# worm-privacy/proof-of-burn

Measured on NVIDIA H100. Metric: main_proof_of_burn witnesses/sec, higher is better.
Workload: dtype u256 (BN254-Fr integer)

## Files before the change

proof-of-burn_b200/csrc/compiler.cpp:

```cpp
#include "compiler.h"
#include <sys/mman.h>
#include <algorithm>
#include <array>
#include <cstdlib>
#include <cstring>
#include <stdexcept>
#include <unordered_map>
#include "poseidon_constants_data.h"
#include "r1cs.h"
#include "vm_exec.h"

namespace pob {
namespace {

struct Blk { uint64_t sig; size_t pos; };
struct Lane { uint32_t w; };

static const Code ZERO = 0, ONE = 1;

struct KeyHash {
    size_t operator()(const std::array<uint32_t, 4> &k) const {
        uint64_t h = 0x9E3779B97F4A7C15ULL;
        for (uint32_t v : k) { h ^= v; h *= 0xBF58476D1CE4E5B9ULL; h ^= h >> 29; }
        return (size_t)h;
// ... 2003 lines not shown
        for (size_t i = 0; i < B.flat_n; i++) B.flat[i] = rc(B.flat[i]);
    }
    std::vector<uint32_t> round_keep;
    if (opt_level) {
        const uint64_t N = B.nsig;
        EqClasses E = eq_classes(P, N);
        const uint64_t n_io = 1ull + n_out + n_in;
        auto kept = [&](uint64_t s) { if (s < n_io) return true; const uint32_t r = E.root((uint32_t)s); return r == s && !E.is_const_root[r]; };
        if (!B.round_sigs.empty()) { const uint64_t b0 = B.round_sigs[0]; for (uint32_t i = 0; i < ROUND_SIGNALS; i++) if (kept(b0 + i)) round_keep.push_back(i); }
        P.witness_map.reserve(N / 8);
        for (auto &sg : B.segs) {
            if (sg.round) {
                size_t k = 0;
                for (uint32_t i = 0; i < ROUND_SIGNALS; i++) {
                    const bool kp = kept(sg.dst + i);
                    const bool want = k < round_keep.size() && round_keep[k] == i;
                    if (kp != want) throw std::runtime_error("pob: internal: KeccakfRound blocks do not reduce uniformly");
                    if (kp) { P.witness_map.push_back((uint32_t)(sg.dst + i)); k++; }
                }
            } else for (uint64_t i = 0; i < sg.n; i++) if (kept(sg.dst + i)) P.witness_map.push_back((uint32_t)(sg.dst + i));
        }
    }
    P.codes.resize(ROUND_SIGNALS);
    { LaneSink S{P.codes.data(), 0}; emit_round(S);
      if ((size_t)(S.p - P.codes.data()) != ROUND_SIGNALS) throw std::runtime_error("pob: internal: round table size mismatch"); }
    P.round_desc = derive_round_desc(P.codes.data(), ROUND_SIGNALS);
    P.n_round_blocks = B.n_round_blocks; P.n_flat_signals = B.flat_n; P.n_signals_o0 = B.nsig; P.opt_level = opt_level;
    if (opt_level) {
        std::vector<Code> rt(round_keep.size()); for (size_t k = 0; k < round_keep.size(); k++) rt[k] = P.codes[round_keep[k]];
        P.codes = rt;
        const uint32_t RT = (uint32_t)round_keep.size();
        bool fast_round = true;
        try { P.round_desc = derive_round_desc(rt.data(), RT); } catch (const std::exception &) { fast_round = false; P.round_desc.assign(1, 0); }
        if (P.round_desc.empty()) P.round_desc.assign(1, 0);
        P.out_code_off = RT + 1;
        uint64_t dst = 0; size_t mp = 0;
        const uint32_t ts = TILE_SIGNALS;
        for (auto &sg : B.segs) {
            if (sg.round) {
                const uint32_t rts = (fast_round && RT <= MAX_TILE_SIGNALS) ? RT : ts;
                for (uint32_t done = 0; done < RT; done += rts) { Tile t; t.dst = dst + done; t.n = std::min(rts, RT - done); t.code_off = done; t.ubase = sg.ubase; t.pad = fast_round ? 1 : 0; P.tiles.push_back(t); }
                dst += RT; mp += RT;
            } else {
                const size_t first = P.codes.size();
                while (mp < P.witness_map.size() && P.witness_map[mp] < sg.dst + sg.n) { P.codes.push_back(B.flat[sg.pos + (P.witness_map[mp] - sg.dst)]); mp++; }
                const uint64_t n = P.codes.size() - first;
                for (uint64_t done = 0; done < n; done += ts) { Tile t; t.dst = dst + done; t.n = (uint32_t)std::min<uint64_t>(ts, n - done); t.code_off = (uint32_t)(first + done); t.ubase = 0; t.pad = 0; P.tiles.push_back(t); }
                dst += n;
            }
        }
        if (dst != P.witness_map.size() || mp != P.witness_map.size()) throw std::runtime_error("pob: internal: reduced layout does not add up");
        P.n_signals = dst;
        if (!user_wants_constraints) { P.cons_flat = ConsSet(); P.cons_round = ConsSet(); P.has_constraints = false; }
        std::stable_sort(P.tiles.begin(), P.tiles.end(), [](const Tile &a, const Tile &b) { return a.pad > b.pad; });
        return P;
    }
    P.codes.insert(P.codes.end(), B.flat, B.flat + B.flat_n);
    uint32_t tile_signals = LAYOUT_TILE_SIGNALS;
#ifdef POB_TUNING
    if (const char *v = getenv("POB_TILE_SIGNALS")) { uint32_t t = (uint32_t)atoi(v); if (t >= 128 && t <= TILE_SIGNALS && t % 128 == 0) tile_signals = t; }
#endif
    for (auto &s : B.segs) {
        uint64_t done = 0;
        while (done < s.n) {
            uint32_t n = (uint32_t)std::min<uint64_t>(tile_signals, s.n - done);
            Tile t; t.dst = s.dst + done; t.n = n; t.pad = 0;
            if (s.round) { t.code_off = (uint32_t)done; t.ubase = s.ubase; t.pad = 1; }
            else { t.code_off = (uint32_t)(ROUND_SIGNALS + s.pos + done); t.ubase = 0; }
            P.tiles.push_back(t); done += n;
        }
    }
    std::stable_sort(P.tiles.begin(), P.tiles.end(), [](const Tile &a, const Tile &b) { return a.pad > b.pad; });
    return P;
}

static uint64_t lc_key(uint32_t idx, bool rel) { return idx == CONS_ONE ? 0 : rel ? (uint64_t)idx + 1 : idx; }
static uint64_t lc_idx(uint64_t key, bool rel) { return !rel ? key : key == 0 ? CONS_ONE : key - 1; }
static LC lc_of(const ConsTerm *t, uint32_t n, const std::vector<Fr> &konst, bool rel) {
    LC L; for (uint32_t i = 0; i < n; i++) L.sf(lc_key(t[i].idx, rel), cons_coef_value(t[i].coef, konst.data(), 0)); return L;
}
static void lc_normalize(LC &L) {
    std::sort(L.t.begin(), L.t.end(), [](const std::pair<uint64_t, Fr> &x, const std::pair<uint64_t, Fr> &y) { return x.first < y.first; });
    size_t o = 0;
    for (size_t i = 0; i < L.t.size();) {
        std::pair<uint64_t, Fr> m = L.t[i++];
        while (i < L.t.size() && L.t[i].first == m.first) m.second = fr_add(m.second, L.t[i++].second);
        if (!fr_is_zero(m.second)) L.t[o++] = m;
    }
    L.t.resize(o);
}
static void lc_unkey(LC &L, bool rel) { for (auto &q : L.t) q.first = lc_idx(q.first, rel); }
static bool plan_r1(ConsSink &S, LC &A, LC &Bq, LC &C, bool rel) {
    lc_normalize(A); lc_normalize(Bq); lc_normalize(C);
    if (A.t.empty()) Bq.t.clear();
    if (A.t.empty() && C.t.empty()) return false;
    lc_unkey(A, rel); lc_unkey(Bq, rel); lc_unkey(C, rel);
    S.r1(A, Bq, C);
    return true;
}

static void plan_o0_set(const ConsSet &in, ConsSink &S, bool rel) {
    const std::vector<Fr> &konst = *S.konst;
    for (size_t i = 0; i + 1 < in.eq.size(); i += 2) if (in.eq[i] != in.eq[i + 1]) S.eq(in.eq[i], in.eq[i + 1]);
    for (const ConsTerm &t : in.kc) {
        const bool on_one = t.idx == CONS_ONE || (!rel && t.idx == 0);
        if (on_one && cc_kind(t.coef) != CC_RCBIT && fr_eq(cons_coef_value(t.coef, konst.data(), 0), fr_from_u64(1))) continue;
        S.kc_raw(t.idx, t.coef);
    }
    for (const ConsR1 &r : in.r1) {
        if (r1_hint(r)) continue;
        const ConsTerm *t = in.terms.data() + r.off;
        LC A = lc_of(t, r.na, konst, rel), Bq = lc_of(t + r.na, r.nb, konst, rel), C = lc_of(t + r.na + r.nb, r1_nc(r), konst, rel);
        plan_r1(S, A, Bq, C, rel);
    }
}

static uint64_t plan_set_terms(const ConsSet &S, const std::vector<Fr> &konst, bool rel, uint64_t rc) {
    uint64_t n = S.eq.size();
    for (const ConsTerm &t : S.kc) {
        const bool on_one = t.idx == CONS_ONE || (!rel && t.idx == 0);
        n += (on_one || fr_is_zero(cons_coef_value(t.coef, konst.data(), rc))) ? 1 : 2;
    }
    for (const ConsR1 &r : S.r1) n += r.na + r.nb + r1_nc(r);
    return n;
}
// ... 127 lines not shown
```

proof-of-burn_b200/csrc/kernels.cuh:

```cuda
#pragma once
#include <cuda_runtime.h>
#include "vm_exec.h"
#include "cons_check.h"

using namespace pob;

namespace {

__constant__ uint64_t c_keccak_rc[24] = {
    0x0000000000000001ULL, 0x0000000000008082ULL, 0x800000000000808AULL, 0x8000000080008000ULL, 0x000000000000808BULL,
    0x0000000080000001ULL, 0x8000000080008081ULL, 0x8000000000008009ULL, 0x000000000000008AULL, 0x0000000000000088ULL,
    0x0000000080008009ULL, 0x000000008000000AULL, 0x000000008000808BULL, 0x800000000000008BULL, 0x8000000000008089ULL,
    0x8000000000008003ULL, 0x8000000000008002ULL, 0x8000000000000080ULL, 0x000000000000800AULL, 0x800000008000000AULL,
    0x8000000080008081ULL, 0x8000000000008080ULL, 0x0000000080000001ULL, 0x8000000080008008ULL};
__constant__ int c_keccak_rot[25] = {1, 10, 7, 11, 17, 18, 3, 5, 16, 8, 21, 24, 4, 15, 23, 19, 13, 12, 2, 20, 14, 22, 9, 6, 1};
__constant__ int c_keccak_inv_rot[25] = {0, 23, 17, 5, 11, 6, 22, 1, 8, 21, 0, 2, 16, 15, 19, 12, 7, 3, 4, 14, 18, 9, 20, 13, 10};

__device__ void absorb_warp(uint64_t *W, const AbsorbOp op) {
    const unsigned FULL = 0xffffffffu;
    const int lane = threadIdx.x & 31;
    const bool act = lane < 25;
    const int l = act ? lane : 0;
    uint64_t st = (act && op.s_idx != NONE_IDX) ? W[op.s_idx + l] : 0ull;
    if (lane < 17) st ^= W[op.blk_idx + lane];
// ... 216 lines not shown
            for (; i < L.t_end; i += GT) {
                const Op cur = nxt;
                if (i + GT < L.t_end) { nxt = ldg_op(a.ops + i + GT); if (a.prefetch) prefetch_operands(x, nxt); }
                vm_exec_op(x, cur);
            }
        }
        for (uint32_t q = L.p_begin + gwarp; q < L.p_end; q += nwarp) poseidon_warp(x, a.poseidons[q], s_pk);
        { const uint32_t np = (L.p_end - L.p_begin) % nwarp, wv = (gwarp + nwarp - np) % nwarp;
          for (uint32_t w = L.w_begin + wv; w < L.w_end; w += nwarp) absorb_warp(U, a.absorbs[w]);
          const uint32_t nw2 = (np + (L.w_end - L.w_begin)) % nwarp, sv = (gwarp + nwarp - nw2) % nwarp;
          for (uint32_t q = L.s_begin + sv; q < L.s_end; q += nwarp) psum_warp(x, a.psums[q]); }
        if (inv_worker) {
            if (lv == a.ginv_level) {
                InvChain c;
                if (vm_ginv_start(x, a.ops, a.ginv_begin, a.inv_end, wid, NWK, c)) { inv_park(s_inv, INV_WORKERS, wt, c); inv_running = true; }
            } else if (inv_running) {
                InvChain c = inv_unpark(s_inv, INV_WORKERS, wt);
                if (inv_chain_steps(c, INV_STEPS)) { vm_ginv_finish(x, a.ops, a.ginv_begin, a.inv_end, wid, NWK, inv_chain_result(c)); inv_running = false; }
                else inv_park(s_inv, INV_WORKERS, wt, c);
            }
        }
        cluster_sync_all();
    }
    if (a.prof && inst == 0 && gt == 0) a.prof[a.n_levels] = clock64();
    if (inv_worker) {
        if (a.ginv_level >= a.n_levels) vm_inv_batch(x, a.ops, a.ginv_begin, a.inv_end, wid, NWK);
        else if (inv_running) {
            InvChain c = inv_unpark(s_inv, INV_WORKERS, wt);
            while (!inv_chain_steps(c, 64)) { }
            vm_ginv_finish(x, a.ops, a.ginv_begin, a.inv_end, wid, NWK, inv_chain_result(c));
        }
    }
    if (a.prof && inst == 0) { cluster_sync_all(); if (gt == 0) { a.prof[a.n_levels + 1] = clock64(); a.prof[a.n_levels + 2] = clock64(); } }
    __syncthreads();
    if (tid == 0 && s_status != STATUS_OK) atomicMin(a.status + inst, s_status);
    cluster_sync_all();
    if (gt == 0 && atomicAdd(a.status + inst, 0u) == STATUS_OK) a.status[inst] = 0u;
    for (uint32_t i = gt; i < a.n_outputs; i += GT) {
        uint64_t v[4]; vm_expand(a.out_codes[i], U, 0, a.val_base, a.konst, v);
        uint64_t *o = a.outputs + ((uint64_t)inst * a.n_outputs + i) * 4;
        o[0] = v[0]; o[1] = v[1]; o[2] = v[2]; o[3] = v[3];
    }
}

__device__ __forceinline__ void st128(uint64_t *p, uint64_t a, uint64_t b) { asm volatile("st.global.v2.b64 [%0], {%1, %2};" ::"l"(p), "l"(a), "l"(b)); }

struct ExpandArgs {
    const Tile *tiles; const Code *codes; const Fr *konst; const uint2 *round_desc;
    const uint64_t *stores; uint64_t store_stride; uint32_t val_base;
    uint64_t *const *wit;
    const uint32_t *inst;
    const uint32_t *status;
    uint32_t chunk_first;
    uint32_t tile0;
};

constexpr int ROUND_THREADS = 256;
__global__ void __launch_bounds__(ROUND_THREADS) k_expand_round(const ExpandArgs a) {
    const uint32_t gi = a.inst[blockIdx.y];
    if (a.status[gi] != 0) return;
    const Tile t = a.tiles[blockIdx.x];
    const uint64_t *Ub = a.stores + (uint64_t)(gi - a.chunk_first) * a.store_stride + t.ubase;
    uint64_t *W = a.wit[blockIdx.y] + t.dst * 4;
    __shared__ __align__(16) uint2 sD[MAX_TILE_SIGNALS / 64];
    __shared__ __align__(16) uint64_t sWraw[ROUND_WORDS_SPAN + 3];
    __shared__ __align__(8) uint64_t s_bar;
    const uint32_t odd = (uint32_t)((reinterpret_cast<uintptr_t>(Ub) >> 3) & 1u);
    const uint32_t nd = (t.n + 63) >> 6, d_bytes = ((nd + 1) & ~1u) * 8u, w_bytes = (ROUND_WORDS_SPAN + 3) / 2 * 16u;
    if (threadIdx.x == 0) mbar_init(&s_bar, 1);
    __syncthreads();
    if (threadIdx.x == 0) {
        mbar_expect_tx(&s_bar, d_bytes + w_bytes);
        tma_load_1d(sD, a.round_desc + (t.code_off >> 6), d_bytes, &s_bar);
        tma_load_1d(sWraw, Ub - odd, w_bytes, &s_bar);
    }
    mbar_wait(&s_bar, 0);
    const uint64_t *sW = sWraw + odd;
#pragma unroll 8
    for (uint32_t u = threadIdx.x; u < 2 * t.n; u += ROUND_THREADS) {
        const uint32_t k = u >> 1;
        const uint2 d = sD[k >> 6];
        const uint32_t tt = k & 63, mode = d.y >> 16;
        uint32_t w = d.x & 0xffffu, b = tt;
        if (mode) {
            const uint32_t sidx = (mode - 1) * 64 + tt, g = sidx / 3, m = sidx - 3 * g;
            b = g; w = (m == 0) ? (d.x & 0xffffu) : (m == 1) ? (d.x >> 16) : (d.y & 0xffffu);
        }
        const uint64_t v = (u & 1u) ? 0ull : (sW[w] >> b) & 1ull;
        st128(W + 2ull * u, v, 0);
    }
}

__global__ void __launch_bounds__(256, 3) k_expand_codes(const ExpandArgs a) {
    constexpr int UG = 4;
    const uint32_t gi = a.inst[blockIdx.x];
    if (a.status[gi] != 0) return;
    const Tile t = a.tiles[a.tile0 + blockIdx.y];
    const uint64_t *U = a.stores + (uint64_t)(gi - a.chunk_first) * a.store_stride;
    uint64_t *W = a.wit[blockIdx.x] + t.dst * 4;
    const uint64_t *Ub = U + t.ubase;
    __shared__ __align__(16) Code sC[TILE_SIGNALS + 4];
    __shared__ __align__(8) uint64_t s_bar;
    const uint32_t off4 = t.code_off & 3u, bytes = (((t.n + off4) * 4u) + 15u) & ~15u;
    if (threadIdx.x == 0) mbar_init(&s_bar, 1);
    __syncthreads();
    if (threadIdx.x == 0) { mbar_expect_tx(&s_bar, bytes); tma_load_1d(sC, a.codes + (t.code_off - off4), bytes, &s_bar); }
    mbar_wait(&s_bar, 0);
    const Code *c = sC + off4;
    const uint32_t n2 = 2 * t.n, h = threadIdx.x & 1u;
    for (uint32_t base = threadIdx.x; base < n2; base += 256 * UG) {
        uint64_t v[UG][2];
#pragma unroll
        for (int j = 0; j < UG; j++) {
            const uint32_t u = base + 256 * j;
            const Code cd = u < n2 ? c[u >> 1] : 0u;
            const uint32_t kind = code_kind(cd), p = code_payload(cd);
            v[j][0] = v[j][1] = 0;
            if (kind == K_VAL || kind == K_KONST) {
                const uint64_t *s = (kind == K_VAL) ? U + a.val_base + 4ull * p : reinterpret_cast<const uint64_t *>(a.konst + p);
                const ulonglong2 q = reinterpret_cast<const ulonglong2 *>(s)[h];
                v[j][0] = q.x; v[j][1] = q.y;
            } else if (!h) v[j][0] = (kind == K_BIT) ? (Ub[p >> 6] >> (p & 63)) & 1ull : p;
        }
#pragma unroll
        for (int j = 0; j < UG; j++) { const uint32_t u = base + 256 * j; if (u < n2) st128(W + 2ull * u, v[j][0], v[j][1]); }
    }
}

__global__ void __launch_bounds__(256) k_digest(const uint64_t *wit, uint64_t n_signals, unsigned long long *out, const uint32_t *status) {
    if (status && *status != 0) return;
    uint64_t acc = 0;
    for (uint64_t i = (uint64_t)blockIdx.x * blockDim.x + threadIdx.x; i < n_signals; i += (uint64_t)gridDim.x * blockDim.x) {
        const ulonglong4 v = *reinterpret_cast<const ulonglong4 *>(wit + 4 * i);
        uint64_t h = (i + 1) * 0x9E3779B97F4A7C15ULL;
        h ^= v.x * 0xBF58476D1CE4E5B9ULL + v.y * 0x94D049BB133111EBULL + v.z * 0xD6E8FEB86659FD93ULL + v.w * 0xA0761D6478BD642FULL;
        h ^= h >> 29; h *= 0xBF58476D1CE4E5B9ULL; h ^= h >> 32;
        acc += h;
    }
    for (int o = 16; o > 0; o >>= 1) acc += __shfl_down_sync(0xffffffffu, acc, o);
    __shared__ uint64_t part[8];
    if ((threadIdx.x & 31) == 0) part[threadIdx.x >> 5] = acc;
    __syncthreads();
    if (threadIdx.x == 0) { uint64_t s = 0; for (int w = 0; w < 8; w++) s += part[w]; atomicAdd(out, (unsigned long long)s); }
}

struct GrindArgs { uint64_t start[4], lanes_tail[9]; uint64_t first, count; uint32_t zero_bytes; unsigned long long *hit; };
__device__ __forceinline__ uint64_t bswap64(uint64_t x) { return __byte_perm((uint32_t)(x >> 32), 0, 0x0123) | ((uint64_t)__byte_perm((uint32_t)x, 0, 0x0123) << 32); }
__device__ __forceinline__ uint64_t rotl64(uint64_t x, int n) { return (x << n) | (x >> (64 - n)); }
__global__ void __launch_bounds__(256) k_pow_grind(const GrindArgs a) {
    const uint64_t idx = (uint64_t)blockIdx.x * blockDim.x + threadIdx.x;
    if (idx >= a.count) return;
    uint64_t k0 = a.start[0], k1 = a.start[1], k2 = a.start[2], k3 = a.start[3];
    const uint64_t add = a.first + idx;
    k0 += add; if (k0 < add) { if (++k1 == 0) { if (++k2 == 0) ++k3; } }
    uint64_t s[25];
    s[0] = bswap64(k3); s[1] = bswap64(k2); s[2] = bswap64(k1); s[3] = bswap64(k0);
#pragma unroll
    for (int i = 0; i < 9; i++) s[4 + i] = a.lanes_tail[i];
    s[13] = 0x01; s[14] = 0; s[15] = 0; s[16] = 0x8000000000000000ull;
#pragma unroll
    for (int i = 17; i < 25; i++) s[i] = 0;
#pragma unroll 1
    for (int r = 0; r < 24; r++) {
        uint64_t c[5], d[5], b[25];
#pragma unroll
        for (int x = 0; x < 5; x++) c[x] = s[x] ^ s[x + 5] ^ s[x + 10] ^ s[x + 15] ^ s[x + 20];
#pragma unroll
        for (int x = 0; x < 5; x++) d[x] = c[(x + 4) % 5] ^ rotl64(c[(x + 1) % 5], 1);
#pragma unroll
        for (int i = 0; i < 25; i++) s[i] ^= d[i % 5];
        b[0] = s[0];
#pragma unroll
        for (int i = 0; i < 24; i++) b[keccak_rot(i + 1)] = rotl64(s[keccak_rot(i)], keccak_shl(i));
#pragma unroll
        for (int i = 0; i < 25; i++) s[i] = b[i] ^ (~b[chi_b(i)] & b[chi_c(i)]);
        s[0] ^= c_keccak_rc[r];
    }
    const uint64_t mask = a.zero_bytes >= 8 ? ~0ull : ((1ull << (8 * a.zero_bytes)) - 1);
    if ((s[0] & mask) == 0) atomicMin(a.hit, (unsigned long long)idx);
// ... 112 lines not shown
```

proof-of-burn_b200/csrc/pob_b200.cu:

```cuda
#include <cuda.h>
#include <cuda_runtime.h>
#include <fcntl.h>
#include <unistd.h>
#include <algorithm>
#include <chrono>
#include <condition_variable>
#include <cstdio>
#include <cstdlib>
#include <cstring>
#include <deque>
#include <mutex>
#include <stdexcept>
#include <string>
#include <thread>
#include <vector>
#include "../../include/pob_b200.h"
#include "compiler.h"
#include "kernels.cuh"
#include "ntt.cuh"
#include "r1cs.h"

using namespace pob;

static thread_local std::string g_err;
// ... 87 lines not shown
        }
    }
    int grab() {
        std::unique_lock<std::mutex> l(m);
        const int b = next_b; cv.wait(l, [&] { return !busy[b]; });
        busy[b] = true; next_b = (b + 1) % NB; return b;
    }
    void drain() { std::unique_lock<std::mutex> l(m); cv.wait(l, [this] { if (!q.empty()) return false; for (int i = 0; i < NB; i++) if (busy[i]) return false; return true; }); }
    static size_t header(uint8_t *o, uint64_t n) {
        uint32_t u32; uint64_t u64; Fr p = fr_p(); size_t k = 0;
        auto put = [&](const void *s, size_t b) { memcpy(o + k, s, b); k += b; };
        put("wtns", 4); u32 = 2; put(&u32, 4); u32 = 2; put(&u32, 4);
        u32 = 1; put(&u32, 4); u64 = 40; put(&u64, 8); u32 = 32; put(&u32, 4); put(p.l, 32); u32 = (uint32_t)n; put(&u32, 4);
        u32 = 2; put(&u32, 4); u64 = 32ull * n; put(&u64, 8);
        return k;
    }
    void send(const uint64_t *dwit, uint64_t n_signals, int fd) {
        CU(cudaSetDevice(device));
        if (fd >= 0) { uint8_t hd[80]; size_t hb = header(hd, n_signals); if (pwrite(fd, hd, hb, 0) != (ssize_t)hb) { std::lock_guard<std::mutex> l(m); io_err = true; } }
        const uint64_t total = 32ull * n_signals; const uint64_t nch = (total + bb - 1) / bb;
        for (uint64_t c = 0; c < nch; c++) {
            const uint64_t off = c * bb; const size_t bytes = (size_t)std::min<uint64_t>(bb, total - off);
            const int b = grab(); cudaStream_t s = cs[rr++ % NS];
            CU(cudaMemcpyAsync(buf[b], (const char *)dwit + off, bytes, cudaMemcpyDeviceToHost, s));
            CU(cudaEventRecord(ev[b], s));
            { std::lock_guard<std::mutex> l(m); q.push_back(Job{b, fd, 76 + off, bytes, c + 1 == nch}); }
            cv.notify_all();
            bytes_moved += bytes;
        }
        if (nch == 0 && fd >= 0) close(fd);
        for (int i = 1; i < NS; i++) { CU(cudaEventRecord(ev_join, cs[i])); CU(cudaStreamWaitEvent(cs[0], ev_join, 0)); }
    }
};

}

struct pob_handle {
    Program P; int device = 0; uint32_t n_sms = 0;
    Op *d_ops = nullptr; PsumOp *d_psums = nullptr; PoseidonOp *d_pos = nullptr; Fr *d_pos_konst = nullptr; AbsorbOp *d_abs = nullptr; Level *d_levels = nullptr; Code *d_aux = nullptr; Fr *d_konst = nullptr;
    Code *d_codes = nullptr; Tile *d_tiles = nullptr; Fr *d_invtab = nullptr; uint64_t *d_round_desc = nullptr;
    static const uint32_t RING = 2;
    uint32_t chunk = 0; uint64_t store_stride = 0; uint64_t *d_stores = nullptr; uint64_t *d_inputs = nullptr;
    std::vector<uint64_t *> slots;
    std::vector<VmSlot> slot_vm; size_t slot_bytes = 0; uint32_t n_compressed_slots = 0;
    std::vector<int64_t> slot_owner;
    std::vector<cudaEvent_t> slot_rel_ev; std::vector<uint8_t> slot_rel_pending;
    std::vector<uint32_t> last_status; uint32_t last_n = 0;
    uint32_t cap_n = 0; uint32_t *d_status = nullptr; uint64_t *d_outputs = nullptr; unsigned long long *d_digests = nullptr;
    uint64_t **d_witptr = nullptr; uint32_t *d_planinst = nullptr;
    uint32_t *h_status = nullptr; uint64_t *h_outputs = nullptr; uint64_t *h_digests = nullptr; uint64_t **h_witptr = nullptr; uint32_t *h_planinst = nullptr;
    uint64_t *d_staged = nullptr; uint32_t n_staged = 0;
    long long *d_prof = nullptr; std::string prof_path;
    uint32_t xgroup = 0;
    uint32_t n_round_tiles = 0;
    uint64_t *d_block_base = nullptr; uint32_t n_blocks = 0;
    uint32_t round_dyn_smem = 85 * 1024;
    uint32_t codes_dyn_smem = 24 * 1024;
    int eval_threads = 512; uint32_t eval_cluster = 0, eval_prefetch = 0;
    uint32_t pos_konst_bytes = 0, levels_bytes = 0, eval_smem = 0;
    bool skip_eval = false;
    cudaStream_t s_eval = nullptr, s_exp = nullptr, s_h2d = nullptr;
    cudaEvent_t ev_eval_done[RING] = {nullptr, nullptr}, ev_exp_done[RING] = {nullptr, nullptr}, ev_h2d[RING] = {nullptr, nullptr},
                ev_start = nullptr, ev_end = nullptr, ev_tmp = nullptr;
    std::vector<cudaEvent_t> ev_pool; size_t ev_used = 0;
    struct Group { uint32_t begin, end, chunk; cudaEvent_t t0, t1; };
    struct Batch {
        bool active = false, async = false, staged = false, digest = false;
        const uint64_t *inputs = nullptr; uint32_t n = 0, nchunks = 0, next_eval = 0, next_group = 0, acq_pos = 0;
        std::vector<uint32_t> plan, slot;
        std::vector<uint8_t> st;
        std::vector<cudaStream_t> acq_stream;
        std::vector<uint32_t> group_of;
        std::vector<Group> groups; std::vector<uint32_t> chunk_gend;
        std::vector<cudaEvent_t> e0, e1, est;
        pob_timing T{};
    } B;
    Exporter *exporter = nullptr;
    pob_timing timing{};
    struct DevCons {
        bool ready = false; ConsView flat{}, round{}; Fr *konst = nullptr; uint64_t *bases = nullptr; uint32_t n_blocks = 0;
        unsigned long long *rep = nullptr; std::vector<void *> allocs; pob_check_report info{};
    } cons, r1cs;
    struct DevNtt { bool ready = false; uint32_t log_n = 0; NttTables t{}; std::vector<void *> allocs; } ntt;
};

static void cons_info(const Program &P, pob_check_report *r) {
    memset(r, 0, sizeof *r);
    const uint64_t nb = P.round_block_sig.size();
    auto count = [&](const ConsSet &S, uint64_t mult) {
        r->n_constraints += mult * (S.eq.size() / 2 + S.kc.size());
        for (const ConsR1 &q : S.r1) { if (r1_hint(q)) r->n_hints += mult; else { r->n_constraints += mult; if (q.na) r->n_nonlinear += mult; } }
    };
    count(P.cons_flat, 1); count(P.cons_round, nb);
    std::vector<uint8_t> seen(P.n_signals, 0);
    auto mark = [&](const ConsSet &S, uint64_t base) {
        for (uint32_t i : S.eq) seen[base + i] = 1;
        for (const ConsTerm &t : S.kc) seen[base + t.idx] = 1;
        for (const ConsTerm &t : S.terms) if (t.idx != CONS_ONE) seen[base + t.idx] = 1;
    };
    mark(P.cons_flat, 0);
    for (uint64_t b : P.round_block_sig) mark(P.cons_round, b);
    for (uint8_t v : seen) r->signals_read += v;
    r->first_failed = ~0ull;
}
static ConsView upload_cons(pob_handle::DevCons &C, const ConsSet &S) {
    ConsView v{};
    auto up = [&](const void *src, size_t bytes) { void *d = nullptr; CU(cudaMalloc(&d, std::max<size_t>(16, bytes))); if (bytes) CU(cudaMemcpy(d, src, bytes, cudaMemcpyHostToDevice)); C.allocs.push_back(d); return d; };
    v.eq = (const uint32_t *)up(S.eq.data(), S.eq.size() * 4); v.n_eq = S.eq.size() / 2;
    v.kc = (const ConsTerm *)up(S.kc.data(), S.kc.size() * sizeof(ConsTerm)); v.n_kc = S.kc.size();
    v.r1 = (const ConsR1 *)up(S.r1.data(), S.r1.size() * sizeof(ConsR1)); v.n_r1 = S.r1.size();
// ... 49 lines not shown
    const uint64_t *d_in;
    if (B.staged) d_in = h->d_staged + (size_t)first * in_stride;
    else {
        uint64_t *dst = h->d_inputs + (size_t)r * E * in_stride;
        if (c >= R) CU(cudaStreamWaitEvent(h->s_h2d, h->ev_eval_done[r], 0));
        if (in_stride) { CU(cudaMemcpyAsync(dst, B.inputs + (size_t)first * in_stride, (size_t)cnt * in_stride * 8, cudaMemcpyHostToDevice, h->s_h2d)); B.T.h2d_bytes += (uint64_t)cnt * in_stride * 8; }
        CU(cudaEventRecord(h->ev_h2d[r], h->s_h2d));
        CU(cudaStreamWaitEvent(h->s_eval, h->ev_h2d[r], 0));
        d_in = dst;
    }
    if (c >= R) CU(cudaStreamWaitEvent(h->s_eval, h->ev_exp_done[r], 0));
    uint64_t *stores = h->d_stores + (size_t)r * E * h->store_stride;
    EvalArgs ea{h->d_ops, h->d_abs, h->d_pos, h->d_pos_konst, h->d_psums, h->d_levels, (uint32_t)P.levels.size(), P.inv_begin, P.ginv_begin, P.inv_end, h->d_aux, h->d_konst, h->d_invtab,
                h->d_codes + P.out_code_off, P.n_outputs, P.n_inputs, P.val_base, stores, h->store_stride, d_in,
                h->d_status + first, h->d_outputs + (size_t)first * no * 4, (c == 0) ? h->d_prof : nullptr, h->pos_konst_bytes, h->levels_bytes, h->eval_prefetch, P.ginv_level};
    CU(cudaEventRecord(B.e0[c], h->s_eval));
    {
        uint32_t C = h->eval_cluster;
        if (C == 0) { C = 8; while (C > 1 && cnt * C > h->n_sms) C >>= 1; }
        cudaLaunchConfig_t cfg{}; cudaLaunchAttribute at[1];
        cfg.gridDim = dim3(cnt * C); cfg.blockDim = dim3((unsigned)h->eval_threads); cfg.dynamicSmemBytes = h->eval_smem; cfg.stream = h->s_eval;
        at[0].id = cudaLaunchAttributeClusterDimension; at[0].val.clusterDim.x = C; at[0].val.clusterDim.y = 1; at[0].val.clusterDim.z = 1;
        cfg.attrs = at; cfg.numAttrs = 1;
        B.T.eval_clusters |= 1u << C;
        if (h->skip_eval && c >= R) CU(cudaMemsetAsync(h->d_status + first, 0, (size_t)cnt * 4, h->s_eval));
        else switch (h->eval_threads) {
        case 256: CU(cudaLaunchKernelEx(&cfg, k_eval<256>, ea)); break;
        case 512: CU(cudaLaunchKernelEx(&cfg, k_eval<512>, ea)); break;
        default: CU(cudaLaunchKernelEx(&cfg, k_eval<1024>, ea)); break;
        }
    }
    CU(cudaEventRecord(B.e1[c], h->s_eval));
    CU(cudaEventRecord(h->ev_eval_done[r], h->s_eval));
    B.T.eval_launches++;
    CU(cudaMemcpyAsync(h->h_status + first, h->d_status + first, (size_t)cnt * 4, cudaMemcpyDeviceToHost, h->s_eval));
    B.T.d2h_bytes += (uint64_t)cnt * 4;
    if (P.n_outputs) { CU(cudaMemcpyAsync(h->h_outputs + (size_t)first * no * 4, h->d_outputs + (size_t)first * no * 4, (size_t)cnt * no * 32, cudaMemcpyDeviceToHost, h->s_eval)); B.T.d2h_bytes += (uint64_t)cnt * no * 32; }
    CU(cudaEventRecord(B.est[c], h->s_eval));
    const uint32_t g0 = c ? B.chunk_gend[c - 1] : 0;
    if (B.chunk_gend[c] == g0) CU(cudaEventRecord(h->ev_exp_done[r], h->s_eval));
}

static void enqueue_group(pob_handle *h, uint32_t g) {
    pob_handle::Batch &B = h->B; const Program &P = h->P;
    const pob_handle::Group &G = B.groups[g];
    const uint32_t E = h->chunk, R = pob_handle::RING, r = G.chunk % R, gc = G.end - G.begin;
    CU(cudaStreamWaitEvent(h->s_exp, h->ev_eval_done[r], 0));
    for (uint32_t k = G.begin; k < G.end; k++) {
        const uint32_t s = B.slot[k];
        if (h->slot_rel_pending[s]) { CU(cudaStreamWaitEvent(h->s_exp, h->slot_rel_ev[s], 0)); h->slot_rel_pending[s] = 0; }
        h->slot_owner[s] = (int64_t)B.plan[k];
    }
    ExpandArgs xa{h->d_tiles, h->d_codes, h->d_konst, reinterpret_cast<const uint2 *>(h->d_round_desc), h->d_stores + (size_t)r * E * h->store_stride, h->store_stride, P.val_base,
                  h->d_witptr + G.begin, h->d_planinst + G.begin, h->d_status, G.chunk * E, 0};
    CU(cudaEventRecord(G.t0, h->s_exp));
    const uint32_t n_round = h->n_round_tiles, n_code = (uint32_t)P.tiles.size() - n_round;
    if (n_round) k_expand_round<<<dim3(n_round, gc), ROUND_THREADS, h->round_dyn_smem, h->s_exp>>>(xa);
    if (n_code) {
        xa.tile0 = n_round;
        k_expand_codes<<<dim3(gc, n_code), 256, h->codes_dyn_smem, h->s_exp>>>(xa);
        B.T.other_launches++;
    }
    CU(cudaEventRecord(G.t1, h->s_exp));
    B.T.expand_launches++;
    if (B.digest) for (uint32_t k = G.begin; k < G.end; k++) {
        k_digest<<<h->n_sms * 8, 256, 0, h->s_exp>>>(h->slots[B.slot[k]], P.n_signals, h->d_digests + B.plan[k], h->d_status + B.plan[k]);
        B.T.other_launches++;
    }
    if (!B.async) for (uint32_t k = G.begin; k < G.end; k++) B.st[k] = 2;
    if (g + 1 == B.chunk_gend[G.chunk]) CU(cudaEventRecord(h->ev_exp_done[r], h->s_exp));
}

static bool group_slots_free(const pob_handle *h, uint32_t g) {
    const pob_handle::Batch &B = h->B; const uint32_t ns = (uint32_t)h->slots.size();
    for (uint32_t k = B.groups[g].begin; k < B.groups[g].end; k++) if (k >= ns && B.st[k - ns] != 2) return false;
    return true;
}
static void advance(pob_handle *h) {
    pob_handle::Batch &B = h->B; const uint32_t R = pob_handle::RING, ng = (uint32_t)B.groups.size();
    for (;;) {
        bool progressed = false;
        if (B.next_eval < B.nchunks && (B.next_eval < R || B.next_group >= B.chunk_gend[B.next_eval - R])) { enqueue_eval(h, B.next_eval++); progressed = true; }
        if (B.next_group < ng && B.groups[B.next_group].chunk < B.next_eval && group_slots_free(h, B.next_group)) { enqueue_group(h, B.next_group++); progressed = true; }
        if (!progressed) break;
    }
    CU(cudaGetLastError());
}

static int begin_batch(pob_handle *h, const uint64_t *inputs, uint32_t n, uint32_t flags, const uint32_t *retain, uint32_t n_retain, bool async, const char *who) {
    const bool staged = (flags & POB_RUN_INPUTS_STAGED) != 0, digest = (flags & POB_RUN_DIGEST) != 0;
    const bool expand = async || (flags & (POB_RUN_EXPAND | POB_RUN_DIGEST)) != 0 || retain != nullptr;
    if (h->B.active) return fail(POB_E_BUSY, std::string(who) + ": a batch is in flight on this handle (pob_finish it first)");
    if (staged ? (h->n_staged < n) : (inputs == nullptr && h->P.n_inputs)) return fail(POB_E_BAD_ARG, std::string(who) + ": no inputs");
    const uint32_t ns = (uint32_t)h->slots.size();
    if (retain) {
        if (n_retain > ns) return fail(POB_E_RANGE, std::string(who) + ": more retained instances than witness slots");
        for (uint32_t k = 0; k < n_retain; k++) if (retain[k] >= n || (k && retain[k] <= retain[k - 1])) return fail(POB_E_BAD_ARG, std::string(who) + ": retain[] must be strictly ascending instance indices");
    } else if (expand && !async && n > ns && !(flags & (POB_RUN_DIGEST | POB_RUN_DISCARD)))
        return fail(POB_E_RANGE, std::string(who) + ": n exceeds the resident witness slots; earlier witnesses would be overwritten unread -- use pob_submit/pob_acquire/pob_release, a retain list, POB_RUN_DIGEST or POB_RUN_DISCARD");
    CU(cudaSetDevice(h->device));
    ensure_batch_buffers(h, n);
    pob_handle::Batch &B = h->B;
    B = pob_handle::Batch();
    B.async = async; B.staged = staged; B.digest = digest; B.inputs = inputs; B.n = n;
    const uint32_t E = h->chunk;
    B.nchunks = (n + E - 1) / E;
    const uint32_t X = async ? std::max<uint32_t>(1, std::min(h->xgroup, ns / 2 ? ns / 2 : 1)) : h->xgroup;
    if (expand) {
        if (retain) B.plan.assign(retain, retain + n_retain);
        else { B.plan.resize(n); for (uint32_t i = 0; i < n; i++) B.plan[i] = i; }
    }
    const uint32_t np = (uint32_t)B.plan.size();
    B.slot.resize(np); B.st.assign(np, 0); B.acq_stream.assign(np, nullptr); B.group_of.resize(np);
    for (uint32_t k = 0; k < np; k++) { B.slot[k] = k % ns; h->h_witptr[k] = h->slots[B.slot[k]]; h->h_planinst[k] = B.plan[k]; }
    h->ev_used = 0;
// ... 120 lines not shown
    for (void *p : h->r1cs.allocs) cudaFree(p);
    for (void *p : h->ntt.allocs) cudaFree(p);
    if (h->s_eval) cudaStreamSynchronize(h->s_eval);
    if (h->s_exp) cudaStreamSynchronize(h->s_exp);
    if (h->s_h2d) cudaStreamSynchronize(h->s_h2d);
    for (void *p : {(void *)h->d_ops, (void *)h->d_psums, (void *)h->d_pos, (void *)h->d_pos_konst, (void *)h->d_abs, (void *)h->d_levels, (void *)h->d_aux, (void *)h->d_konst, (void *)h->d_codes,
                    (void *)h->d_tiles, (void *)h->d_invtab, (void *)h->d_round_desc, (void *)h->d_stores, (void *)h->d_inputs, (void *)h->d_status,
                    (void *)h->d_outputs, (void *)h->d_digests, (void *)h->d_witptr, (void *)h->d_planinst, (void *)h->d_staged, (void *)h->d_prof, (void *)h->d_block_base})
        if (p) cudaFree(p);
    if (!h->slot_vm.empty()) {
        const DriverVmm &D = vmm();
        cudaDeviceSynchronize();
        for (const VmSlot &s : h->slot_vm) {
            if (s.mapped) D.unmap(s.va, h->slot_bytes);
            if (s.va) D.addressFree(s.va, h->slot_bytes);
            if (s.mem) D.release(s.mem);
        }
    }
    for (void *p : {(void *)h->h_status, (void *)h->h_outputs, (void *)h->h_digests, (void *)h->h_witptr, (void *)h->h_planinst}) if (p) cudaFreeHost(p);
    for (cudaEvent_t e : h->ev_pool) cudaEventDestroy(e);
    for (cudaEvent_t e : h->slot_rel_ev) cudaEventDestroy(e);
    for (uint32_t r = 0; r < pob_handle::RING; r++) {
        if (h->ev_eval_done[r]) cudaEventDestroy(h->ev_eval_done[r]);
        if (h->ev_exp_done[r]) cudaEventDestroy(h->ev_exp_done[r]);
        if (h->ev_h2d[r]) cudaEventDestroy(h->ev_h2d[r]);
    }
    for (cudaEvent_t e : {h->ev_start, h->ev_end, h->ev_tmp}) if (e) cudaEventDestroy(e);
    for (cudaStream_t s : {h->s_h2d, h->s_eval, h->s_exp}) if (s) cudaStreamDestroy(s);
    delete h;
}

int pob_create(const char *main_name, const uint64_t *params, int nparams, int hcreate, int device, uint32_t max_slots, pob_handle **out) {
    if (!main_name || !out || (nparams > 0 && !params)) return fail(POB_E_BAD_ARG, "pob_create: null argument");
    *out = nullptr;
    int ndev = 0;
    if (cudaGetDeviceCount(&ndev) != cudaSuccess || ndev == 0) return fail(POB_E_NO_DEVICE, "pob_create: no CUDA device (this library has no CPU path)");
    if (device < 0 || device >= ndev) return fail(POB_E_NO_DEVICE, "pob_create: device index out of range");
    pob_handle *h = new pob_handle(); h->device = device;
    try { h->P = compile_circuit(main_name, params_vec(params, nparams), flag_hcreate(hcreate), false, flag_opt(hcreate)); }
    catch (const std::exception &e) { delete h; return fail(POB_E_COMPILE, e.what()); }
    try {
        const Program &P = h->P;
        CU(cudaSetDevice(device));
        { int v = 0; CU(cudaDeviceGetAttribute(&v, cudaDevAttrMultiProcessorCount, device)); h->n_sms = (uint32_t)v; }
        h->d_ops = upload(P.ops); h->d_psums = upload(P.psums); h->d_pos = upload(P.poseidons); h->d_pos_konst = upload(P.pos_konst); h->d_abs = upload(P.absorbs); h->d_levels = upload(P.levels); h->d_aux = upload(P.aux);
        h->pos_konst_bytes = (uint32_t)(P.pos_konst.size() * sizeof(Fr)); h->levels_bytes = (uint32_t)(std::max<size_t>(1, P.levels.size()) * sizeof(Level));
        h->d_konst = upload(P.konst);
        { std::vector<Code> cd = P.codes; cd.resize(cd.size() + 8, 0); h->d_codes = upload(cd); }
        if (const char *v = tune_env("POB_TILE_FILTER")) {
            std::vector<Tile> sub; for (const Tile &t : P.tiles) if ((atoi(v) == 1) == (t.pad != 0)) sub.push_back(t);
            h->P.tiles = sub;
        }
        h->d_tiles = upload(h->P.tiles);
        for (const Tile &t : h->P.tiles) if (t.pad) h->n_round_tiles++;
        { std::vector<uint64_t> bases; for (const Tile &t : P.tiles) if (t.pad && t.code_off == 0) bases.push_back(t.dst);
          std::sort(bases.begin(), bases.end()); h->n_blocks = (uint32_t)bases.size(); h->d_block_base = upload(bases); }
        h->d_invtab = upload(build_inverse_table());
        { std::vector<uint64_t> rd = P.round_desc; rd.resize(rd.size() + 2, 0); h->d_round_desc = upload(rd); }
        int pr_least = 0, pr_greatest = 0; CU(cudaDeviceGetStreamPriorityRange(&pr_least, &pr_greatest));
        CU(cudaStreamCreateWithPriority(&h->s_eval, cudaStreamNonBlocking, pr_greatest));
        CU(cudaStreamCreateWithPriority(&h->s_h2d, cudaStreamNonBlocking, pr_greatest));
        CU(cudaStreamCreateWithPriority(&h->s_exp, cudaStreamNonBlocking, pr_least));
        for (uint32_t r = 0; r < pob_handle::RING; r++) {
            CU(cudaEventCreateWithFlags(&h->ev_eval_done[r], cudaEventDisableTiming));
            CU(cudaEventCreateWithFlags(&h->ev_exp_done[r], cudaEventDisableTiming));
            CU(cudaEventCreateWithFlags(&h->ev_h2d[r], cudaEventDisableTiming));
        }
        CU(cudaEventCreate(&h->ev_start)); CU(cudaEventCreate(&h->ev_end)); CU(cudaEventCreateWithFlags(&h->ev_tmp, cudaEventDisableTiming));
        if (const char *v = tune_env("POB_EVAL_PROFILE")) { h->prof_path = v; CU(cudaMalloc(&h->d_prof, (P.levels.size() + 3) * sizeof(long long))); }
        size_t free_b = 0, total_b = 0; CU(cudaMemGetInfo(&free_b, &total_b));
        const uint64_t wbytes = 32ull * P.n_signals;
        h->store_stride = std::max<uint64_t>(32, (P.store_u64() + 31) & ~31ull);
        uint32_t chunk = (uint32_t)std::min<uint64_t>(1024, std::max<uint64_t>(32, (512ull << 20) / (h->store_stride * 8)));
        if (P.opt_level) chunk = std::max<uint32_t>(chunk, 128);
        chunk -= chunk % 32;
        if (const char *v = tune_env("POB_EVAL_CHUNK")) chunk = (uint32_t)std::max(1, atoi(v));
        const DriverVmm &D = vmm();
        CUdevice cdev = 0; CUD(D.deviceGet(&cdev, device));
        int compress = 0; CUD(D.deviceGetAttribute(&compress, CU_DEVICE_ATTRIBUTE_GENERIC_COMPRESSION_SUPPORTED, cdev));
        if (const char *v = tune_env("POB_SLOT_COMPRESS")) compress = compress && atoi(v) != 0;
        CUmemAllocationProp mprop{};
        mprop.type = CU_MEM_ALLOCATION_TYPE_PINNED; mprop.location.type = CU_MEM_LOCATION_TYPE_DEVICE; mprop.location.id = device;
        mprop.allocFlags.compressionType = compress ? CU_MEM_ALLOCATION_COMP_GENERIC : CU_MEM_ALLOCATION_COMP_NONE;
        size_t gran = 0; CUD(D.granularity(&gran, &mprop, CU_MEM_ALLOC_GRANULARITY_RECOMMENDED));
        const size_t vbytes = (wbytes + gran - 1) / gran * gran;
        const uint64_t ring_bytes_per_inst = pob_handle::RING * (h->store_stride * 8 + (uint64_t)P.n_inputs * 32);
        uint64_t budget = (uint64_t)(free_b * 0.8);
        uint64_t nslots = budget > chunk * ring_bytes_per_inst ? (budget - chunk * ring_bytes_per_inst) / vbytes : 0;
        if (max_slots && nslots > max_slots) nslots = max_slots;
        if (nslots > 4096) nslots = 4096;
        if (nslots == 0) throw std::runtime_error("not even one witness slot fits in free HBM");
        h->chunk = chunk;
        CU(cudaMalloc(&h->d_stores, (size_t)pob_handle::RING * chunk * h->store_stride * 8));
        CU(cudaMalloc(&h->d_inputs, std::max<size_t>(32, (size_t)pob_handle::RING * chunk * P.n_inputs * 32)));
        h->slot_bytes = vbytes;
        CUmemAccessDesc acc{}; acc.location = mprop.location; acc.flags = CU_MEM_ACCESS_FLAGS_PROT_READWRITE;
        for (uint64_t s = 0; s < nslots; s++) {
            CUmemGenericAllocationHandle mem = 0;
            const CUresult r = D.create(&mem, vbytes, &mprop, 0);
            if (r == CUDA_ERROR_OUT_OF_MEMORY && s > 0) break;
            if (r == CUDA_ERROR_OUT_OF_MEMORY) throw std::runtime_error("not even one witness slot fits in free HBM (cuMemCreate)");
            if (r != CUDA_SUCCESS) throw std::runtime_error("cuMemCreate: CUresult " + std::to_string((int)r));
            h->slot_vm.push_back(VmSlot{}); VmSlot &m = h->slot_vm.back(); m.mem = mem;
            CUD(D.reserve(&m.va, vbytes, gran, 0, 0));
            CUD(D.map(m.va, vbytes, 0, m.mem, 0)); m.mapped = true;
            CUD(D.setAccess(m.va, vbytes, &acc, 1));
            CUmemAllocationProp got{}; CUD(D.properties(&got, m.mem));
            if (got.allocFlags.compressionType == CU_MEM_ALLOCATION_COMP_GENERIC) h->n_compressed_slots++;
            h->slots.push_back(reinterpret_cast<uint64_t *>(m.va));
        }
        nslots = h->slots.size();
        h->xgroup = (uint32_t)std::min<uint64_t>(std::min<uint64_t>(nslots, chunk), std::max<uint64_t>(16, (100ull << 30) / wbytes));
        if (const char *v = tune_env("POB_EVAL_THREADS")) h->eval_threads = atoi(v);
        if (const char *v = tune_env("POB_EVAL_CLUSTER")) h->eval_cluster = (uint32_t)std::max(0, std::min(8, atoi(v)));
        if (const char *v = tune_env("POB_EVAL_PREFETCH")) h->eval_prefetch = (uint32_t)(atoi(v) != 0);
        if (const char *v = tune_env("POB_SKIP_EVAL")) h->skip_eval = atoi(v) != 0;
        if (h->eval_threads != 256 && h->eval_threads != 512) h->eval_threads = 1024;
        h->eval_smem = h->pos_konst_bytes + h->levels_bytes + INV_WORKERS * INV_PARK_WORDS * 4u;
        if (h->eval_smem > 200 * 1024) throw std::runtime_error("the Poseidon constant table, the level table and the parked inversions do not fit in shared memory");
        CU(cudaFuncSetAttribute(k_eval<256>, cudaFuncAttributeMaxDynamicSharedMemorySize, (int)h->eval_smem));
        CU(cudaFuncSetAttribute(k_eval<512>, cudaFuncAttributeMaxDynamicSharedMemorySize, (int)h->eval_smem));
        CU(cudaFuncSetAttribute(k_eval<1024>, cudaFuncAttributeMaxDynamicSharedMemorySize, (int)h->eval_smem));
        if (const char *v = tune_env("POB_EXPAND_SMEM_KB")) h->round_dyn_smem = (uint32_t)atoi(v) * 1024u;
        if (const char *v = tune_env("POB_CODES_SMEM_KB")) h->codes_dyn_smem = (uint32_t)atoi(v) * 1024u;
        CU(cudaFuncSetAttribute(k_expand_codes, cudaFuncAttributeMaxDynamicSharedMemorySize, (int)h->codes_dyn_smem));
        if (h->round_dyn_smem > 48 * 1024) CU(cudaFuncSetAttribute(k_expand_round, cudaFuncAttributeMaxDynamicSharedMemorySize, (int)h->round_dyn_smem));
        if (const char *v = tune_env("POB_EXPAND_GROUP")) h->xgroup = (uint32_t)std::max(1, std::min<int>(atoi(v), (int)std::min<uint64_t>(nslots, chunk)));
        h->slot_owner.assign(nslots, -1); h->slot_rel_pending.assign(nslots, 0);
        for (uint64_t s = 0; s < nslots; s++) { cudaEvent_t e; CU(cudaEventCreateWithFlags(&e, cudaEventDisableTiming)); h->slot_rel_ev.push_back(e); }
    } catch (const std::exception &e) {
        std::string m = e.what(); pob_destroy(h);
        return fail(m.find("slot") != std::string::npos ? POB_E_NO_MEMORY : POB_E_CUDA, "pob_create: " + m);
    }
    *out = h; return POB_OK;
}

int pob_witness_map(const pob_handle *h, uint32_t *map) {
    if (!h || !map) return fail(POB_E_BAD_ARG, "pob_witness_map: null argument");
    if (!h->P.opt_level) return fail(POB_E_BAD_ARG, "pob_witness_map: the handle produces the full --O0 witness (identity map)");
    memcpy(map, h->P.witness_map.data(), h->P.witness_map.size() * 4);
    return POB_OK;
}

int pob_describe(const pob_handle *h, pob_desc *out) {
    if (!h || !out) return fail(POB_E_BAD_ARG, "pob_describe: null argument");
    fill_desc(h->P, out); out->n_slots = (uint32_t)h->slots.size(); out->chunk = h->chunk; out->expand_group = h->xgroup;
    out->n_compressed_slots = h->n_compressed_slots; return POB_OK;
}

void *pob_alloc_pinned(uint64_t bytes) { void *p = nullptr; if (cudaMallocHost(&p, bytes ? bytes : 1) != cudaSuccess) { g_err = "cudaMallocHost failed"; return nullptr; } return p; }
void pob_free_pinned(void *p) { if (p) cudaFreeHost(p); }

int pob_stage_inputs(pob_handle *h, const uint64_t *inputs, uint32_t n) {
    if (!h || !inputs || n == 0) return fail(POB_E_BAD_ARG, "pob_stage_inputs: bad argument");
    if (h->B.active) return fail(POB_E_BUSY, "pob_stage_inputs: a batch is in flight");
    try {
        CU(cudaSetDevice(h->device));
        if (h->d_staged) { cudaFree(h->d_staged); h->d_staged = nullptr; h->n_staged = 0; }
        size_t bytes = std::max<size_t>(32, (size_t)n * h->P.n_inputs * 32);
        CU(cudaMalloc(&h->d_staged, bytes));
        if (h->P.n_inputs) CU(cudaMemcpy(h->d_staged, inputs, (size_t)n * h->P.n_inputs * 32, cudaMemcpyHostToDevice));
        h->n_staged = n;
    } catch (const std::exception &e) { return fail(POB_E_CUDA, e.what()); }
    return POB_OK;
}

static int run_batch_impl(pob_handle *h, const uint64_t *inputs, uint32_t n, uint32_t flags, const uint32_t *retain, uint32_t n_retain,
                          uint32_t *status, uint64_t *outputs, uint64_t *digests, const char *who) {
    if (!h || n == 0 || !status) return fail(POB_E_BAD_ARG, std::string(who) + ": bad argument");
    if ((flags & POB_RUN_DIGEST) && !digests) return fail(POB_E_BAD_ARG, std::string(who) + ": POB_RUN_DIGEST needs a digests array");
    try {
        int rc = begin_batch(h, inputs, n, flags, retain, n_retain, false, who);
        if (rc) return rc;
        return finish_batch(h, status, outputs, digests);
    } catch (const std::exception &e) { abort_batch(h); return fail(POB_E_CUDA, std::string(who) + ": " + e.what()); }
}
int pob_run_batch(pob_handle *h, const uint64_t *inputs, uint32_t n, uint32_t flags, uint32_t *status, uint64_t *outputs, uint64_t *digests) {
    return run_batch_impl(h, inputs, n, flags, nullptr, 0, status, outputs, digests, "pob_run_batch");
}
// ... 388 lines not shown
```

Measured before the change: 564.1.

## Merge round and code expand kernels into one launch over all tiles

Replaces the separate round-tile and code-tile expand kernels with a single k_expand kernel that branches per tile on the pad flag. This removes the second launch and the tile sorting by kind. It also folds small trailing round-tile remainders into the previous tile. In exchange every block reserves both the static round buffers and the dynamic code buffer, and launch bounds change from (256,3) to (256,2) for the code path, which may lower occupancy. The grid order for code tiles also changes from instance-major to tile-major.

```diff
diff --git a/proof-of-burn_b200/csrc/compiler.cpp b/proof-of-burn_b200/csrc/compiler.cpp
--- a/proof-of-burn_b200/csrc/compiler.cpp
+++ b/proof-of-burn_b200/csrc/compiler.cpp
@@ -2079,7 +2079,6 @@
         if (dst != P.witness_map.size() || mp != P.witness_map.size()) throw std::runtime_error("pob: internal: reduced layout does not add up");
         P.n_signals = dst;
         if (!user_wants_constraints) { P.cons_flat = ConsSet(); P.cons_round = ConsSet(); P.has_constraints = false; }
-        std::stable_sort(P.tiles.begin(), P.tiles.end(), [](const Tile &a, const Tile &b) { return a.pad > b.pad; });
         return P;
     }
     P.codes.insert(P.codes.end(), B.flat, B.flat + B.flat_n);
@@ -2091,13 +2090,13 @@
         uint64_t done = 0;
         while (done < s.n) {
             uint32_t n = (uint32_t)std::min<uint64_t>(tile_signals, s.n - done);
+            if (s.round && s.n - done - n < tile_signals / 4) n = (uint32_t)(s.n - done);
             Tile t; t.dst = s.dst + done; t.n = n; t.pad = 0;
             if (s.round) { t.code_off = (uint32_t)done; t.ubase = s.ubase; t.pad = 1; }
             else { t.code_off = (uint32_t)(ROUND_SIGNALS + s.pos + done); t.ubase = 0; }
             P.tiles.push_back(t); done += n;
         }
     }
-    std::stable_sort(P.tiles.begin(), P.tiles.end(), [](const Tile &a, const Tile &b) { return a.pad > b.pad; });
     return P;
 }
 
diff --git a/proof-of-burn_b200/csrc/kernels.cuh b/proof-of-burn_b200/csrc/kernels.cuh
--- a/proof-of-burn_b200/csrc/kernels.cuh
+++ b/proof-of-burn_b200/csrc/kernels.cuh
@@ -292,32 +292,24 @@
     const uint32_t *inst;
     const uint32_t *status;
     uint32_t chunk_first;
-    uint32_t tile0;
 };
 
-constexpr int ROUND_THREADS = 256;
-__global__ void __launch_bounds__(ROUND_THREADS) k_expand_round(const ExpandArgs a) {
-    const uint32_t gi = a.inst[blockIdx.y];
-    if (a.status[gi] != 0) return;
-    const Tile t = a.tiles[blockIdx.x];
-    const uint64_t *Ub = a.stores + (uint64_t)(gi - a.chunk_first) * a.store_stride + t.ubase;
-    uint64_t *W = a.wit[blockIdx.y] + t.dst * 4;
-    __shared__ __align__(16) uint2 sD[MAX_TILE_SIGNALS / 64];
-    __shared__ __align__(16) uint64_t sWraw[ROUND_WORDS_SPAN + 3];
-    __shared__ __align__(8) uint64_t s_bar;
+constexpr int EXPAND_THREADS = 256;
+constexpr uint32_t EXPAND_CODE_SMEM = (TILE_SIGNALS + 4) * 4;
+
+__device__ __forceinline__ void expand_round_tile(const Tile &t, const uint2 *round_desc, const uint64_t *Ub, uint64_t *W,
+                                                  uint2 *sD, uint64_t *sWraw, uint64_t *bar) {
     const uint32_t odd = (uint32_t)((reinterpret_cast<uintptr_t>(Ub) >> 3) & 1u);
     const uint32_t nd = (t.n + 63) >> 6, d_bytes = ((nd + 1) & ~1u) * 8u, w_bytes = (ROUND_WORDS_SPAN + 3) / 2 * 16u;
-    if (threadIdx.x == 0) mbar_init(&s_bar, 1);
-    __syncthreads();
     if (threadIdx.x == 0) {
-        mbar_expect_tx(&s_bar, d_bytes + w_bytes);
-        tma_load_1d(sD, a.round_desc + (t.code_off >> 6), d_bytes, &s_bar);
-        tma_load_1d(sWraw, Ub - odd, w_bytes, &s_bar);
-    }
-    mbar_wait(&s_bar, 0);
+        mbar_expect_tx(bar, d_bytes + w_bytes);
+        tma_load_1d(sD, round_desc + (t.code_off >> 6), d_bytes, bar);
+        tma_load_1d(sWraw, Ub - odd, w_bytes, bar);
+    }
+    mbar_wait(bar, 0);
     const uint64_t *sW = sWraw + odd;
 #pragma unroll 8
-    for (uint32_t u = threadIdx.x; u < 2 * t.n; u += ROUND_THREADS) {
+    for (uint32_t u = threadIdx.x; u < 2 * t.n; u += EXPAND_THREADS) {
         const uint32_t k = u >> 1;
         const uint2 d = sD[k >> 6];
         const uint32_t tt = k & 63, mode = d.y >> 16;
@@ -331,28 +323,20 @@
     }
 }
 
-__global__ void __launch_bounds__(256, 3) k_expand_codes(const ExpandArgs a) {
+__device__ __forceinline__ void expand_code_tile(const ExpandArgs &a, const Tile &t, const uint64_t *U, uint64_t *W,
+                                                 Code *sC, uint64_t *bar) {
     constexpr int UG = 4;
-    const uint32_t gi = a.inst[blockIdx.x];
-    if (a.status[gi] != 0) return;
-    const Tile t = a.tiles[a.tile0 + blockIdx.y];
-    const uint64_t *U = a.stores + (uint64_t)(gi - a.chunk_first) * a.store_stride;
-    uint64_t *W = a.wit[blockIdx.x] + t.dst * 4;
     const uint64_t *Ub = U + t.ubase;
-    __shared__ __align__(16) Code sC[TILE_SIGNALS + 4];
-    __shared__ __align__(8) uint64_t s_bar;
     const uint32_t off4 = t.code_off & 3u, bytes = (((t.n + off4) * 4u) + 15u) & ~15u;
-    if (threadIdx.x == 0) mbar_init(&s_bar, 1);
-    __syncthreads();
-    if (threadIdx.x == 0) { mbar_expect_tx(&s_bar, bytes); tma_load_1d(sC, a.codes + (t.code_off - off4), bytes, &s_bar); }
-    mbar_wait(&s_bar, 0);
+    if (threadIdx.x == 0) { mbar_expect_tx(bar, bytes); tma_load_1d(sC, a.codes + (t.code_off - off4), bytes, bar); }
+    mbar_wait(bar, 0);
     const Code *c = sC + off4;
     const uint32_t n2 = 2 * t.n, h = threadIdx.x & 1u;
-    for (uint32_t base = threadIdx.x; base < n2; base += 256 * UG) {
+    for (uint32_t base = threadIdx.x; base < n2; base += EXPAND_THREADS * UG) {
         uint64_t v[UG][2];
 #pragma unroll
         for (int j = 0; j < UG; j++) {
-            const uint32_t u = base + 256 * j;
+            const uint32_t u = base + EXPAND_THREADS * j;
             const Code cd = u < n2 ? c[u >> 1] : 0u;
             const uint32_t kind = code_kind(cd), p = code_payload(cd);
             v[j][0] = v[j][1] = 0;
@@ -363,8 +347,24 @@
             } else if (!h) v[j][0] = (kind == K_BIT) ? (Ub[p >> 6] >> (p & 63)) & 1ull : p;
         }
 #pragma unroll
-        for (int j = 0; j < UG; j++) { const uint32_t u = base + 256 * j; if (u < n2) st128(W + 2ull * u, v[j][0], v[j][1]); }
-    }
+        for (int j = 0; j < UG; j++) { const uint32_t u = base + EXPAND_THREADS * j; if (u < n2) st128(W + 2ull * u, v[j][0], v[j][1]); }
+    }
+}
+
+__global__ void __launch_bounds__(EXPAND_THREADS, 2) k_expand(const ExpandArgs a) {
+    extern __shared__ __align__(128) uint8_t dyn_smem[];
+    __shared__ __align__(16) uint2 sD[MAX_TILE_SIGNALS / 64];
+    __shared__ __align__(16) uint64_t sWraw[ROUND_WORDS_SPAN + 3];
+    __shared__ __align__(8) uint64_t s_bar;
+    const uint32_t gi = a.inst[blockIdx.y];
+    if (a.status[gi] != 0) return;
+    const Tile t = a.tiles[blockIdx.x];
+    const uint64_t *U = a.stores + (uint64_t)(gi - a.chunk_first) * a.store_stride;
+    uint64_t *W = a.wit[blockIdx.y] + t.dst * 4;
+    if (threadIdx.x == 0) mbar_init(&s_bar, 1);
+    __syncthreads();
+    if (t.pad) expand_round_tile(t, a.round_desc, U + t.ubase, W, sD, sWraw, &s_bar);
+    else expand_code_tile(a, t, U, W, reinterpret_cast<Code *>(dyn_smem), &s_bar);
 }
 
 __global__ void __launch_bounds__(256) k_digest(const uint64_t *wit, uint64_t n_signals, unsigned long long *out, const uint32_t *status) {
diff --git a/proof-of-burn_b200/csrc/pob_b200.cu b/proof-of-burn_b200/csrc/pob_b200.cu
--- a/proof-of-burn_b200/csrc/pob_b200.cu
+++ b/proof-of-burn_b200/csrc/pob_b200.cu
@@ -163,10 +163,8 @@
     uint64_t *d_staged = nullptr; uint32_t n_staged = 0;
     long long *d_prof = nullptr; std::string prof_path;
     uint32_t xgroup = 0;
-    uint32_t n_round_tiles = 0;
     uint64_t *d_block_base = nullptr; uint32_t n_blocks = 0;
-    uint32_t round_dyn_smem = 85 * 1024;
-    uint32_t codes_dyn_smem = 24 * 1024;
+    uint32_t expand_dyn_smem = 85 * 1024;
     int eval_threads = 512; uint32_t eval_cluster = 0, eval_prefetch = 0;
     uint32_t pos_konst_bytes = 0, levels_bytes = 0, eval_smem = 0;
     bool skip_eval = false;
@@ -322,15 +320,9 @@
         h->slot_owner[s] = (int64_t)B.plan[k];
     }
     ExpandArgs xa{h->d_tiles, h->d_codes, h->d_konst, reinterpret_cast<const uint2 *>(h->d_round_desc), h->d_stores + (size_t)r * E * h->store_stride, h->store_stride, P.val_base,
-                  h->d_witptr + G.begin, h->d_planinst + G.begin, h->d_status, G.chunk * E, 0};
+                  h->d_witptr + G.begin, h->d_planinst + G.begin, h->d_status, G.chunk * E};
     CU(cudaEventRecord(G.t0, h->s_exp));
-    const uint32_t n_round = h->n_round_tiles, n_code = (uint32_t)P.tiles.size() - n_round;
-    if (n_round) k_expand_round<<<dim3(n_round, gc), ROUND_THREADS, h->round_dyn_smem, h->s_exp>>>(xa);
-    if (n_code) {
-        xa.tile0 = n_round;
-        k_expand_codes<<<dim3(gc, n_code), 256, h->codes_dyn_smem, h->s_exp>>>(xa);
-        B.T.other_launches++;
-    }
+    if (!P.tiles.empty()) k_expand<<<dim3((uint32_t)P.tiles.size(), gc), EXPAND_THREADS, h->expand_dyn_smem, h->s_exp>>>(xa);
     CU(cudaEventRecord(G.t1, h->s_exp));
     B.T.expand_launches++;
     if (B.digest) for (uint32_t k = G.begin; k < G.end; k++) {
@@ -557,7 +549,6 @@
             h->P.tiles = sub;
         }
         h->d_tiles = upload(h->P.tiles);
-        for (const Tile &t : h->P.tiles) if (t.pad) h->n_round_tiles++;
         { std::vector<uint64_t> bases; for (const Tile &t : P.tiles) if (t.pad && t.code_off == 0) bases.push_back(t.dst);
           std::sort(bases.begin(), bases.end()); h->n_blocks = (uint32_t)bases.size(); h->d_block_base = upload(bases); }
         h->d_invtab = upload(build_inverse_table());
@@ -626,10 +617,8 @@
         CU(cudaFuncSetAttribute(k_eval<256>, cudaFuncAttributeMaxDynamicSharedMemorySize, (int)h->eval_smem));
         CU(cudaFuncSetAttribute(k_eval<512>, cudaFuncAttributeMaxDynamicSharedMemorySize, (int)h->eval_smem));
         CU(cudaFuncSetAttribute(k_eval<1024>, cudaFuncAttributeMaxDynamicSharedMemorySize, (int)h->eval_smem));
-        if (const char *v = tune_env("POB_EXPAND_SMEM_KB")) h->round_dyn_smem = (uint32_t)atoi(v) * 1024u;
-        if (const char *v = tune_env("POB_CODES_SMEM_KB")) h->codes_dyn_smem = (uint32_t)atoi(v) * 1024u;
-        CU(cudaFuncSetAttribute(k_expand_codes, cudaFuncAttributeMaxDynamicSharedMemorySize, (int)h->codes_dyn_smem));
-        if (h->round_dyn_smem > 48 * 1024) CU(cudaFuncSetAttribute(k_expand_round, cudaFuncAttributeMaxDynamicSharedMemorySize, (int)h->round_dyn_smem));
+        if (const char *v = tune_env("POB_EXPAND_SMEM_KB")) h->expand_dyn_smem = std::max((uint32_t)atoi(v) * 1024u, EXPAND_CODE_SMEM);
+        CU(cudaFuncSetAttribute(k_expand, cudaFuncAttributeMaxDynamicSharedMemorySize, (int)h->expand_dyn_smem));
         if (const char *v = tune_env("POB_EXPAND_GROUP")) h->xgroup = (uint32_t)std::max(1, std::min<int>(atoi(v), (int)std::min<uint64_t>(nslots, chunk)));
         h->slot_owner.assign(nslots, -1); h->slot_rel_pending.assign(nslots, 0);
         for (uint64_t s = 0; s < nslots; s++) { cudaEvent_t e; CU(cudaEventCreateWithFlags(&e, cudaEventDisableTiming)); h->slot_rel_ev.push_back(e); }
```

Measured after the change: 566.8, median of 6. No clear change (+0.5%).
